# tkkiran/Robust-Conditional-GAN

Hardware: AMD Instinct MI355X
Metric: images/sec G+D train step (CIFAR-10 RCGAN bs=64) (higher is better)
Workload: dtype bf16

## Files before the change

### include/rcgan_hip.h

```cpp
#ifndef RCGAN_HIP_H
#define RCGAN_HIP_H

#include <stddef.h>
#include <stdint.h>

#ifdef __cplusplus
extern "C" {
#endif

#define RCGAN_OK 0
#define RCGAN_EINVALID_ARG (-1)
#define RCGAN_EUNSUPPORTED_SHAPE (-2)
#define RCGAN_EWORKSPACE_TOO_SMALL (-3)
#define RCGAN_EHIP (-4)
#define RCGAN_ERCCL (-5)

#define RCGAN_F32 0
#define RCGAN_BF16 1
#define RCGAN_F16 2

#define RCGAN_ACT_NONE 0
#define RCGAN_ACT_RELU 1
#define RCGAN_ACT_LRELU 2
#define RCGAN_ACT_TANH 3
// ... 217 lines not shown
int rcgan_dtrunk_prepare(rcgan_ctx* ctx, const void* const* prepared, void* frag);
int rcgan_dtrunk(rcgan_ctx* ctx, int n, int backward, const void* x0, const void* frag, const float* const* bias,
                 const void* const* masks, void* const* outs);
int rcgan_dtrunk_pooled(rcgan_ctx* ctx, int n, int backward, const void* x0, const void* frag, const float* const* bias,
                        const void* const* masks, void* const* outs, float* feat, const void* xlast, void* dy_out);

int rcgan_conv_rf_ok(const rcgan_conv_desc* d);
size_t rcgan_conv_rf_fragment_bytes(const rcgan_conv_desc* d);
int rcgan_conv_rf_prepare(rcgan_ctx* ctx, int n, const rcgan_conv_desc* descs, const void* const* prepared, void* const* frags);
int rcgan_fragments_prepare(rcgan_ctx* ctx, const void* const* trunk_prepared, void* trunk_frag, int n, const rcgan_conv_desc* descs,
                            const void* const* prepared, void* const* frags);
int rcgan_conv2d_rf(rcgan_ctx* ctx, const rcgan_conv_desc* d, int backward, const void* x, const void* frag, const float* bias,
                    const void* mask_x, const void* residual, void* y);

int rcgan_dblock2_ok(const rcgan_conv_desc* d, const void* conv1_frag, const void* dblock2_frag);
size_t rcgan_dblock2_fragment_bytes(void);
int rcgan_fragments_prepare_dblock2(rcgan_ctx* ctx, const void* const* trunk_prepared, void* trunk_frag, int n, const rcgan_conv_desc* descs,
                                    const void* const* prepared, void* const* frags, const void* conv2_prepared,
                                    const void* shortcut_prepared, void* dblock2_frag);
int rcgan_dblock2_fwd(rcgan_ctx* ctx, const rcgan_conv_desc* d, const void* x, const void* conv1_frag, const void* dblock2_frag,
                      const float* bias1, const float* bias2, const float* bias_shortcut, void* h, void* xp, void* y);
int rcgan_dblock2_bwd(rcgan_ctx* ctx, const rcgan_conv_desc* d, const void* dy, const void* h, const void* x, const void* conv1_frag,
                      const void* dblock2_frag, void* dh, void* dx);
size_t rcgan_proj_head_workspace_bytes(int n, int d, int v);
typedef struct {
  int n, d, v, e_dim;
  int rows_a, kind_a, kind_b;
  float weight;
  const int32_t* labels_a; const float* wts_a; float* dwts_a;
  const int32_t* labels_b; const float* wts_b; float* dwts_b;
  const void* x; void* dx;
  int x_dtype, hw, act;
  const float* E_pre;
  void* defer_ws;
  size_t defer_ws_bytes;
} rcgan_head_desc;
int rcgan_proj_head_fwd_bwd(rcgan_ctx* ctx, const rcgan_head_desc* hd, const float* feat, const float* w_out, const float* sigma_out,
                            const float* b_out, const float* table, const float* w_e, const float* sigma_e, const float* b_e,
                            float* loss_acc, float* logits, float* dfeat, float* dw_out, float* db_out, float* dtable, float* dw_e,
                            float* db_e, void* ws, size_t ws_bytes);
int rcgan_head_flush(rcgan_ctx* ctx);
int rcgan_bce_onehot_fwd_bwd(rcgan_ctx* ctx, int rows, int cols, const float* x, const int32_t* labels,
                             float weight, float* loss_acc, float* dx);
size_t rcgan_recover_mse_workspace_bytes(int r, int ydim);
int rcgan_recover_mse_fwd_bwd(rcgan_ctx* ctx, int r, int ydim, int pix, int dtype, const void* gen, const void* actual,
                              const float* yrec, float* loss, void* dgen, float* dyrec, void* ws, size_t ws_bytes);
// ... 116 lines not shown
```

### robust-conditional-gan_amd/_lib.py

```python
import ctypes as C
import os

_HERE = os.path.dirname(os.path.abspath(__file__))
LIB_PATH = os.environ.get("RCGAN_LIB_PATH") or os.path.join(_HERE, "librcgan_hip.so")
LIB_PATH_F16 = os.environ.get("RCGAN_LIB_PATH_F16") or os.path.join(_HERE, "librcgan_hip_f16.so")

F32, BF16, F16 = 0, 1, 2
ACT_NONE, ACT_RELU, ACT_LRELU, ACT_TANH, ACT_SIGMOID = 0, 1, 2, 3, 4
CONV_IN_UPSAMPLE2X, CONV_IN_RELU, CONV_ACCUMULATE, CONV_FORCE_DIRECT, CONV_OUT_MEANPOOL2, CONV_RESID_UPSAMPLE2X = 1, 2, 4, 8, 16, 32
LOSS_HINGE_REAL, LOSS_HINGE_FAKE, LOSS_NEG_MEAN, LOSS_CE_ONES, LOSS_CE_ZEROS = 0, 1, 2, 3, 4
QUERY_TR_READ = 0
AUG_COLOR, AUG_TRANSLATION, AUG_CUTOUT = 1, 2, 4
AUG_POLICIES = {"color": AUG_COLOR, "translation": AUG_TRANSLATION, "cutout": AUG_CUTOUT}
F32_PRECISION_HIGHEST, F32_PRECISION_HIGH = 0, 1
F32_PRECISIONS = {"highest": F32_PRECISION_HIGHEST, "high": F32_PRECISION_HIGH}

RCGAN_EHIP, RCGAN_ERCCL = -4, -5
EINVALID_ARG, EUNSUPPORTED_SHAPE, EWORKSPACE_TOO_SMALL = -1, -2, -3
ERRORS = {-1: "RCGAN_EINVALID_ARG", -2: "RCGAN_EUNSUPPORTED_SHAPE", -3: "RCGAN_EWORKSPACE_TOO_SMALL",
          -4: "RCGAN_EHIP", -5: "RCGAN_ERCCL"}


def source_hash():
    import glob
# ... 164 lines not shown
    "rcgan_act_meanhw_fwd": (I, [P, I, I, I, I, I, P, P]),
    "rcgan_act_meanhw_bwd": (I, [P, I, I, I, I, I, P, P, P]),
    "rcgan_gather_rows": (I, [P, I, I, P, P, P]),
    "rcgan_scatter_add_rows": (I, [P, I, I, I, P, P, P, I]),
    "rcgan_proj_logit_fwd": (I, [P, I, I, P, P, P, P]),
    "rcgan_proj_logit_bwd": (I, [P, I, I, P, P, P, P, P, P, I]),
    "rcgan_proj_logit_all_fwd": (I, [P, I, I, I, P, P, P, P]),
    "rcgan_proj_logit_all_bwd": (I, [P, I, I, I, P, P, P, P, P, P, I]),
    "rcgan_loss_fwd_bwd": (I, [P, I, I, I, P, P, F, P, P, P]),
    "rcgan_bce_onehot_fwd_bwd": (I, [P, I, I, P, P, F, P, P]),
    "rcgan_dtrunk": (I, [P, I, I, P, P, P, P, P]),
    "rcgan_dtrunk_pooled": (I, [P, I, I, P, P, P, P, P, P, P, P]),
    "rcgan_dtrunk_prepare": (I, [P, P, P]),
    "rcgan_conv_rf_ok": (I, [C.POINTER(ConvDesc)]),
    "rcgan_conv_rf_fragment_bytes": (SZ, [C.POINTER(ConvDesc)]),
    "rcgan_conv_rf_prepare": (I, [P, I, C.POINTER(ConvDesc), P, P]),
    "rcgan_fragments_prepare": (I, [P, P, P, I, C.POINTER(ConvDesc), P, P]),
    "rcgan_conv2d_rf": (I, [P, C.POINTER(ConvDesc), I, P, P, P, P, P, P]),
    "rcgan_dblock2_ok": (I, [C.POINTER(ConvDesc), P, P]),
    "rcgan_dblock2_fragment_bytes": (SZ, []),
    "rcgan_fragments_prepare_dblock2": (I, [P, P, P, I, C.POINTER(ConvDesc), P, P, P, P, P]),
    "rcgan_dblock2_fwd": (I, [P, C.POINTER(ConvDesc), P, P, P, P, P, P, P, P, P]),
    "rcgan_dblock2_bwd": (I, [P, C.POINTER(ConvDesc), P, P, P, P, P, P, P]),
    "rcgan_dtrunk_fragment_bytes": (SZ, []),
    "rcgan_head_flush": (I, [P]),
    "rcgan_proj_head_fwd_bwd": (I, [P, C.POINTER(HeadDesc)] + [P] * 16 + [P, SZ]),
    "rcgan_recover_mse_fwd_bwd": (I, [P, I, I, I, I, P, P, P, P, P, P, P, SZ]),
    "rcgan_softmax_rows_fwd": (I, [P, I, I, P, P]),
    "rcgan_softmax_rows_bwd": (I, [P, I, I, P, P, P, I]),
    "rcgan_softmax_xent_workspace_bytes": (SZ, [I]),
    "rcgan_softmax_xent_fwd_bwd": (I, [P, I, I, P, P, F, P, P, P, P, SZ]),
    "rcgan_softmax_xent_forward_fwd_bwd": (I, [P, I, I, P, P, P, F, P, P, P, P, P, P, SZ]),
    "rcgan_shortcut_a_fwd": (I, [P, I, I, I, I, I, P, P]),
    "rcgan_shortcut_a_bwd": (I, [P, I, I, I, I, I, P, P, I]),
    "rcgan_diffaugment_fwd": (I, [P, I, I, I, I, I, P, P, P, P]),
    "rcgan_diffaugment_bwd": (I, [P, I, I, I, I, I, P, P, P, I]),
    "rcgan_diffaugment_gated_fwd": (I, [P, I, I, I, I, I, P, P, P, P, P, P, P]),
    "rcgan_diffaugment_sampled_bwd": (I, [P, I, I, I, I, P, P, P, P, I]),
    "rcgan_ada_update": (I, [P, I, P, I, P, P, F, F, I]),
    "rcgan_class_moments_bytes": (SZ, [I, I]),
    "rcgan_class_moments_accum": (I, [P, I, I, I, P, P, P]),
    "rcgan_knn_radius": (I, [P, I, I, I, I, P, P, P]),
    "rcgan_ball_query": (I, [P, I, I, I, I, P, P, P, P, P, P, P]),
    "rcgan_poly3_rowsum": (I, [P, I, I, I, I, P, P, P, P, C.c_double, C.c_double, I, P]),
    "rcgan_msssim_pairs": (I, [P, I, I, I, I, I, P, P, P]),
    "rcgan_nn_u8": (I, [P, I, I, I, I, P, P, P, P, I, P]),
# ... 67 lines not shown
```

### robust-conditional-gan_amd/cifar.py

```python
import ctypes as C
import os

import warnings

import numpy as np
import torch

from . import _lib as L
from . import ops as O
from . import runtime
from .ops_cifar import NO_OPS, Conv2D, Linear, cond_batchnorm, embed_y, spectral_normed_weight
from .runtime import DT, Context, ParamGroup, check_f32_matmul_precision, run_rehearsed
from .variables import Graph, scoped, variable_scope

Z_DIM = 128
DIM_G = 128
DIM_D = 128
VOCAB_SIZE = 10
EMBEDDING_DIM = 300
IMG_SIZE = 32
IMG_DIM = 3
OUTPUT_DIM = 3072
N_CRITIC = 5
GEN_BS_MULTIPLE = 2
# ... 233 lines not shown
                                    _defer_apply=True)
        output = Conv2D(output, DIM_G * 2, IMG_DIM, 3, 1, 'G.Output', he_init=False)
        output = O.act(ctx, output, L.ACT_TANH, out=out.reshape(output.shape) if out is not None else None)
        return O.reshape(ctx, output, (-1, OUTPUT_DIM))


def fused_pool_d(ctx, n):
    if ctx.act_dtype == L.F32 or os.environ.get("RCGAN_FUSED_POOL", "1") != "1":
        return False
    d1 = L.ConvDesc(n, IMG_SIZE, IMG_SIZE, DIM_D, DIM_D, 3, 3, 1, ctx.act_dtype, L.CONV_OUT_MEANPOOL2)
    d2 = L.ConvDesc(n, IMG_SIZE // 2, IMG_SIZE // 2, DIM_D, DIM_D, 3, 3, 1, ctx.act_dtype, L.CONV_OUT_MEANPOOL2)
    return bool(ctx.lib.rcgan_conv_fused_pool_ok(C.byref(d1))) and bool(ctx.lib.rcgan_conv_fused_pool_ok(C.byref(d2)))


def Discriminator(inputs, labels, update_collection=None, _head=True):
    ctx = _ctx()
    kw = dict(spectral_normed=True, update_collection=update_collection)
    with variable_scope("Discriminator"):
        x = O.reshape(ctx, inputs, (-1, IMG_SIZE, IMG_SIZE, IMG_DIM))
        if fused_pool_d(ctx, x.shape[0]):
            xp = getattr(Graph.current, "image_pool", None)
            if xp is not None and (x.req or xp.shape != (x.shape[0], x.shape[1] // 2, x.shape[2] // 2, x.shape[3])):
                xp = None
            t = Conv2D(xp if xp is not None else O.meanpool2(ctx, x), IMG_DIM, DIM_D, 1, 1, 'D.Block.1.Shortcut', he_init=False, **kw)
            h = Conv2D(x, IMG_DIM, DIM_D, 3, 1, 'D.Block.1.Conv1', **kw)
            x = Conv2D(h, DIM_D, DIM_D, 3, 1, 'D.Block.1.Conv2', _in_relu=True, _accumulate_into=t, _out_meanpool=True, **kw)
            g, wb = Graph.current, []
            for cv in ('Shortcut', 'Conv1', 'Conv2'):
                with variable_scope('D.Block.2.%s' % cv):
                    fname = scoped('Filters')
                    with variable_scope('filters'):
                        wb.append(spectral_normed_weight(fname, update_collection=update_collection))
                    wb.append(g.param(scoped('Biases')))
            dfrag = getattr(g, "dblock2_frag", None)
            if O.d_block2_ok(ctx, x, wb[2], dfrag):
                x = O.d_block2(ctx, x, *wb, frag=dfrag)
            else:
                t = O.conv2d(ctx, O.meanpool2(ctx, x), wb[0], wb[1], 1)
                h = O.conv2d(ctx, x, wb[2], wb[3], 3, in_relu=True)
                x = O.conv2d_meanpool(ctx, h, wb[4], wb[5], in_relu=True, accumulate_into=t)
        else:
            t = Conv2D(x, IMG_DIM, DIM_D, 1, 1, 'D.Block.1.Shortcut', he_init=False, **kw)
            h = Conv2D(x, IMG_DIM, DIM_D, 3, 1, 'D.Block.1.Conv1', **kw)
            t = Conv2D(h, DIM_D, DIM_D, 3, 1, 'D.Block.1.Conv2', _in_relu=True, _accumulate_into=t, **kw)
            x = O.meanpool2(ctx, t)
            t = Conv2D(x, DIM_D, DIM_D, 1, 1, 'D.Block.2.Shortcut', he_init=False, **kw)
            h = Conv2D(x, DIM_D, DIM_D, 3, 1, 'D.Block.2.Conv1', _in_relu=True, **kw)
            t = Conv2D(h, DIM_D, DIM_D, 3, 1, 'D.Block.2.Conv2', _in_relu=True, _accumulate_into=t, **kw)
            x = O.meanpool2(ctx, t)
        if Graph.current.early_d is not None and x.req:
# ... 314 lines not shown
        for n in grp.names:
            if n.endswith("/Filters"):
                shp = grp.shapes[n]
                up = L.CONV_IN_UPSAMPLE2X if (n.startswith("Generator/G.Block.") and n.endswith(".Conv1/Filters")) else 0
                if pool and n in ("Discriminator/D.Block.1.Conv2/Filters", "Discriminator/D.Block.2.Conv2/Filters"):
                    up = L.CONV_OUT_MEANPOOL2
                names.append((n, shp[0], 1, IMG_SIZE if min(shp[2], shp[3]) <= 3 else 8, up))
            elif n == "Generator/G.Input/W" and O.LINEAR_MFMA:
                names.append((n, 1, 1, 1, 0))
        return names

    def _prepare_all(self, which, head_update=False, inputs=None):
        names = []
        for grp in which:
            if grp is not self.PG:
                names += self._filter_names(grp)
        g, embed = self.graph, None
        g.head_E = None
        if self.fused_head and self.PD in which and head_update is not False and self.K <= L.LABELS_NARROW and \
                os.environ.get("RCGAN_HEAD_EMBED_RIDE", "1") == "1":
            _, _, table, w_e, b_e = _head_weights(head_update)
            E = self.ctx.empty((table.shape[0], w_e.param.shape[-1]), L.F32)
            embed = (table, w_e, b_e, E)
        g.trunk_frag = g.dblock2_frag = None
        trunk, rf, db2 = None, [], None
        if self.PD in which and self.ctx.act_dtype != L.F32 and (FUSED_TRUNK or O.RF_CONV):
            sn = lambda n: g.sn["Discriminator/%s/Filters" % n][0]
            trunk = [sn("D.Block.%d.%s" % (b, c)) for b in (3, 4, 5, 6) for c in ("Conv1", "Conv2")] if FUSED_TRUNK else None
            if O.RF_CONV:
                d = L.ConvDesc(1, 16, 16, DIM_D, DIM_D, 3, 3, 1, self.ctx.act_dtype, L.CONV_IN_RELU)
                if self.ctx.lib.rcgan_conv_rf_ok(C.byref(d)):
                    rf.append((sn("D.Block.2.Conv1"), d))
                    if O.FUSED_DBLOCK2 and fused_pool_d(self.ctx, GEN_BS_MULTIPLE * self.B):
                        db2 = (sn("D.Block.2.Conv2"), sn("D.Block.2.Shortcut"))
        if (trunk or rf) and O.FRAG_IN_PREPARE:
            tf, reqs = O.fragment_requests(self.ctx, trunk, rf)
            rode, written = g.prepare_convs(names, self.ctx.act_dtype, embed=embed, inputs=inputs, frags=reqs)
            if len(written) == len(reqs):
                g.trunk_frag = tf
            else:
                g.trunk_frag = O.fragments_batch(self.ctx, trunk, rf)
        else:
            rode = g.prepare_convs(names, self.ctx.act_dtype, embed=embed, inputs=inputs)
            if db2 is not None:
                g.trunk_frag, g.dblock2_frag = O.fragments_batch(self.ctx, trunk, rf, dblock2=db2)
            elif trunk or rf:
                g.trunk_frag = O.fragments_batch(self.ctx, trunk, rf)
        if rode and embed is not None:
            g.head_E = embed[3]
        return rode

    def _refresh_generator_filters(self):
        if self._pg_prepared_version != self.PG.version:
            self.graph.refresh_persistent(self._filter_names(self.PG), self.ctx.act_dtype)
            self._pg_prepared_version = self.PG.version

    def confusion_matrix(self):
        ctx = self.ctx
        if self.PC is not None:
            return O.softmax_rows(ctx, self.graph.param("confusion_logits"))
        return self.inp["C_const"]

    def _rides_inputs(self):
        return self.device_rng and self.ride_inputs and self.PD.gradbuf.numel() % 4 == 0

    def _d_body(self, fakes_ready=False):
        ctx, g, B, inp = self.ctx, self.graph, self.B, self.inp
# ... 502 lines not shown
```

### robust-conditional-gan_amd/csrc/conv_rf.hip

```cpp
#include <type_traits>

#include "conv_mfma.h"
#include "mfma_util.h"
#include "rf_asm.h"

namespace {

struct RfArgs {
  const bf16_t* in;
  const bf16_t* wfrag;
  const float* bias;
  const bf16_t* mask;
  const bf16_t* resid;
  bf16_t* out;
  const bf16_t* zero;
  int accumulate, relu_in;
  int H, W, lbpi, Cout;
  int res_lw, res_lh;
  long M;
  unsigned long long* stamps;
};

constexpr int RF_ROWS = 8;
constexpr int RF_UPFRONT = 4;
// ... 210 lines not shown
      for (int dir = 0; dir < 2; ++dir) {
        const int K = 9 * (dir ? d->cout : d->cin), nsl = (dir ? d->cout : d->cin) / 64;
        FragItem& it = b.it[2 * i + dir];
        it.src = (const bf16_t*)prepared[i0 + i] + dir * elems;
        it.dst = (bf16_t*)frags[i0 + i] + dir * elems;
        it.K = K; it.ctn = 4; it.ss = 18; it.nsl = nsl; it.chunks = (int)(elems / 8);
        if (it.chunks > maxchunks) maxchunks = it.chunks;
      }
    }
    hipLaunchKernelGGL(rf_fragments_kernel, dim3(cdiv(maxchunks, 256), 2 * m), dim3(256), 0, ctx->stream, b);
    RC_LAUNCH_CHECK(ctx);
  }
  return RCGAN_OK;
}

int rcgan_fragments_prepare(rcgan_ctx* ctx, const void* const* trunk_prepared, void* trunk_frag, int n, const rcgan_conv_desc* descs,
                            const void* const* prepared, void* const* frags) {
  return rcgan_fragments_prepare_dblock2(ctx, trunk_prepared, trunk_frag, n, descs, prepared, frags, nullptr, nullptr, nullptr);
}

int rcgan_fragments_prepare_dblock2(rcgan_ctx* ctx, const void* const* trunk_prepared, void* trunk_frag, int n, const rcgan_conv_desc* descs,
                                    const void* const* prepared, void* const* frags, const void* conv2_prepared,
                                    const void* shortcut_prepared, void* dblock2_frag) {
  if (!ctx) return RCGAN_EINVALID_ARG;
  RC_REQUIRE(ctx, n >= 0 && n <= 12 && (n == 0 || (descs && prepared && frags)) && (!trunk_prepared || trunk_frag), "bad arguments");
  RC_REQUIRE(ctx, (conv2_prepared != nullptr) == (dblock2_frag != nullptr) && (shortcut_prepared != nullptr) == (dblock2_frag != nullptr),
             "the down block's copies need both prepared filters and a destination");
  RC_REQUIRE(ctx, (dblock2_frag ? DB2_FRAG_ITEMS : 0) + (trunk_prepared ? 16 : 0) + 2 * n <= (int)(sizeof(FragBatch::it) / sizeof(FragItem)),
             "more fragment items than one launch holds");
  FragBatch b;
  int m = 0, maxchunks = 0;
  if (dblock2_frag) {
    const rcgan_conv_desc d2 = {1, 16, 16, 128, 128, 3, 3, 1, RCGAN_H16, RCGAN_CONV_OUT_MEANPOOL2};
    const rcgan_conv_desc ds = {1, 8, 8, 128, 128, 1, 1, 1, RCGAN_H16, 0};
    dblock2_frag_items((const bf16_t*)conv2_prepared + mfma_prepared_sum_fwd(&d2), (const bf16_t*)shortcut_prepared,
                       (const bf16_t*)conv2_prepared + mfma_prepared_sum_bwd(&d2), (const bf16_t*)shortcut_prepared + mfma_prepared_rot(&ds),
                       (bf16_t*)dblock2_frag, b.it);
    m = DB2_FRAG_ITEMS;
    maxchunks = b.it[0].chunks;
  }
  if (trunk_prepared) {
    const long elems = 9L * 128 * 128;
    for (int i = 0; i < 8; ++i) {
      RC_REQUIRE(ctx, trunk_prepared[i], "stage layer %d: null pointer", i);
      b.it[m++] = FragItem{(const bf16_t*)trunk_prepared[i], (bf16_t*)trunk_frag + i * elems, 1152, 2, 36, 1, (int)(elems / 8)};
      b.it[m++] = FragItem{(const bf16_t*)trunk_prepared[7 - i] + elems, (bf16_t*)trunk_frag + (8 + i) * elems, 1152, 2, 36, 1, (int)(elems / 8)};
    }
    if ((int)(elems / 8) > maxchunks) maxchunks = (int)(elems / 8);
  }
  for (int i = 0; i < n; ++i) {
    const rcgan_conv_desc* d = descs + i;
    RC_REQUIRE(ctx, rf_takes(d) && prepared[i] && frags[i], "filter %d: not a register-filter shape / null pointer", i);
    const long elems = 9L * d->cin * d->cout;
    for (int dir = 0; dir < 2; ++dir) {
      const int kc = dir ? d->cout : d->cin;
      b.it[m++] = FragItem{(const bf16_t*)prepared[i] + dir * elems, (bf16_t*)frags[i] + dir * elems, 9 * kc, 4, 18, kc / 64, (int)(elems / 8)};
    }
    if ((int)(elems / 8) > maxchunks) maxchunks = (int)(elems / 8);
  }
  if (m == 0) return RCGAN_OK;
  hipLaunchKernelGGL(rf_fragments_kernel, dim3(cdiv(maxchunks, 256), m), dim3(256), 0, ctx->stream, b);
  RC_LAUNCH_CHECK(ctx);
// ... 31 lines not shown
```

### robust-conditional-gan_amd/csrc/rf_asm.h

```cpp
#pragma once
#include <type_traits>

#include "mfma_util.h"

typedef __attribute__((ext_vector_type(4))) int i32x4_t;

#if RCGAN_HALF_FP16
#define RF_MFMA "v_mfma_f32_16x16x32_f16"
#else
#define RF_MFMA "v_mfma_f32_16x16x32_bf16"
#endif

template <int OFF> __device__ __forceinline__ void rf_load_a(i32x4_t& dst, const void* p) {
  asm volatile("global_load_dwordx4 %0, %1, off offset:%2" : "=a"(dst) : "v"(p), "n"(OFF) : "memory");
}
template <int OFF> __device__ __forceinline__ void rf_load_v(i32x4_t& dst, const void* p) {
  asm volatile("global_load_dwordx4 %0, %1, off offset:%2" : "=v"(dst) : "v"(p), "n"(OFF) : "memory");
}
template <int OFF> __device__ __forceinline__ void rf_load_a_inplace(i32x4_t& dst, const void* p) {
  asm volatile("global_load_dwordx4 %0, %1, off offset:%2" : "+a"(dst) : "v"(p), "n"(OFF) : "memory");
}
__device__ __forceinline__ void rf_mfma_a(f32x4_t& acc, const i32x4_t& w, const bf16x8_t& x) {
  asm volatile(RF_MFMA " %0, %1, %2, %0" : "+v"(acc) : "a"(w), "v"(x) : "memory");
}
__device__ __forceinline__ void rf_mfma_v(f32x4_t& acc, const i32x4_t& w, const bf16x8_t& x) {
  asm volatile(RF_MFMA " %0, %1, %2, %0" : "+v"(acc) : "v"(w), "v"(x) : "memory");
}
__device__ __forceinline__ void rf_mfma_a0(f32x4_t& acc, const i32x4_t& w, const bf16x8_t& x) {
  asm volatile(RF_MFMA " %0, %1, %2, 0" : "=v"(acc) : "a"(w), "v"(x) : "memory");
}
__device__ __forceinline__ void rf_lds_read(bf16x8_t& dst, unsigned lds_byte_addr) {
  asm volatile("ds_read_b128 %0, %1" : "=v"(dst) : "v"(lds_byte_addr) : "memory");
}
template <int N> __device__ __forceinline__ void rf_wait() { asm volatile("s_waitcnt vmcnt(%0)" :: "n"(N) : "memory"); }
__device__ __forceinline__ void rf_barrier() { asm volatile("s_waitcnt lgkmcnt(0)\n\ts_barrier" ::: "memory"); }

template <int I, int N, typename F> __device__ __forceinline__ void rf_for(F&& f) {
  if constexpr (I < N) { f(std::integral_constant<int, I>{}); rf_for<I + 1, N>(f); }
}

struct FragItem { const bf16_t* src; bf16_t* dst; int K, ctn, ss, nsl, chunks; };

constexpr long DB2_FRAG_CONV2 = 16L * 128 * 128;
constexpr long DB2_FRAG_SHORT = 128L * 128;
constexpr long DB2_FRAG_CONV2_BWD = DB2_FRAG_CONV2 + DB2_FRAG_SHORT;
constexpr long DB2_FRAG_SHORT_BWD = DB2_FRAG_CONV2_BWD + DB2_FRAG_CONV2;
constexpr long DB2_FRAG_ELEMS = DB2_FRAG_SHORT_BWD + DB2_FRAG_SHORT;
constexpr int DB2_FRAG_ITEMS = 4;
inline void dblock2_frag_items(const bf16_t* conv2_sum_fwd, const bf16_t* shortcut_fwd, const bf16_t* conv2_sum_bwd, const bf16_t* shortcut_rot,
                               bf16_t* frag, FragItem* it) {
  it[0] = FragItem{conv2_sum_fwd, frag, 2048, 2, 64, 1, (int)(DB2_FRAG_CONV2 / 8)};
  it[1] = FragItem{shortcut_fwd, frag + DB2_FRAG_CONV2, 128, 2, 4, 1, (int)(DB2_FRAG_SHORT / 8)};
  it[2] = FragItem{conv2_sum_bwd, frag + DB2_FRAG_CONV2_BWD, 512, 2, 16, 1, (int)(DB2_FRAG_CONV2 / 8)};
  it[3] = FragItem{shortcut_rot, frag + DB2_FRAG_SHORT_BWD, 128, 2, 4, 1, (int)(DB2_FRAG_SHORT / 8)};
}
```

### robust-conditional-gan_amd/ops.py

```python
import ctypes as C
import os

import torch

from . import _lib as L
from .runtime import DT


def _p(t):
    return C.c_void_p(t.ptr) if t is not None else None


def same_pad(n, k, s):
    out = -(-n // s)
    tot = max((out - 1) * s + k - n, 0)
    return out, tot // 2


def zeros_like_grad(ctx, t):
    g = ctx.empty(t.shape, t.dtype)
    ctx.check(ctx.lib.rcgan_fill_f32(ctx.h, (g.nbytes + 3) // 4, g.ptr, 0.0))
    return g


# ... 119 lines not shown
CONCAT_DIRECT = os.environ.get("RCGAN_CONCAT_DIRECT", "1") != "0"
CONCAT_WGRAD = os.environ.get("RCGAN_CONCAT_WGRAD", "1") != "0"
LINEAR_MFMA = os.environ.get("RCGAN_LINEAR_MFMA", "1") != "0"


FRAG_IN_PREPARE = os.environ.get("RCGAN_FRAG_IN_PREPARE", "0") == "1"


def fragment_requests(ctx, trunk, rf):
    reqs, tf = [], None
    if trunk:
        nb = ctx.lib.rcgan_dtrunk_fragment_bytes()
        tf = DT(ctx.arena.alloc(nb), (nb,), "u8", ctx.arena.buf)
        elems2 = 9 * 128 * 128 * 2
        for i, w in enumerate(trunk):
            reqs.append((w, tf.ptr + i * elems2, tf.ptr + (8 + (7 - i)) * elems2, 2, 36))
    for w, d in rf:
        nb = ctx.lib.rcgan_conv_rf_fragment_bytes(C.byref(d))
        w.rf_frag = DT(ctx.arena.alloc(nb), (nb,), "u8", ctx.arena.buf)
        reqs.append((w, w.rf_frag.ptr, w.rf_frag.ptr + nb // 2, 4, 18))
    return tf, reqs


def fragments_batch(ctx, trunk, rf, dblock2=None):
    tp = tf = None
    if trunk:
        tdesc = L.ConvDesc(1, 8, 8, 128, 128, 3, 3, 1, ctx.act_dtype, L.CONV_IN_RELU)
        tp = (C.c_void_p * 8)(*[w.prepared(tdesc).ptr for w in trunk])
        nb = ctx.lib.rcgan_dtrunk_fragment_bytes()
        tf = DT(ctx.arena.alloc(nb), (nb,), "u8", ctx.arena.buf)
    n = len(rf)
    descs = (L.ConvDesc * max(n, 1))(*[d for _, d in rf])
    preps = (C.c_void_p * max(n, 1))(*[w.prepared(d).ptr for w, d in rf])
    frags = []
    for w, d in rf:
        nb = ctx.lib.rcgan_conv_rf_fragment_bytes(C.byref(d))
        w.rf_frag = DT(ctx.arena.alloc(nb), (nb,), "u8", ctx.arena.buf)
        frags.append(w.rf_frag.ptr)
    if dblock2 is not None:
        w2, ws = dblock2
        p2 = w2.prepared(L.ConvDesc(1, 8, 8, 128, 128, 3, 3, 1, ctx.act_dtype, L.CONV_OUT_MEANPOOL2))
        ps = ws.prepared(L.ConvDesc(1, 8, 8, 128, 128, 1, 1, 1, ctx.act_dtype, 0))
        nb = ctx.lib.rcgan_dblock2_fragment_bytes()
        df = DT(ctx.arena.alloc(nb), (nb,), "u8", ctx.arena.buf)
        ctx.check(ctx.lib.rcgan_fragments_prepare_dblock2(ctx.h, tp, _p(tf), n, descs, preps, (C.c_void_p * max(n, 1))(*frags),
                                                          _p(p2), _p(ps), _p(df)))
        return tf, df
    ctx.check(ctx.lib.rcgan_fragments_prepare(ctx.h, tp, _p(tf), n, descs, preps, (C.c_void_p * max(n, 1))(*frags)))
    return tf


def spectral_norm_batch(ctx, entries):
    n = len(entries)
    if n == 0:
        return []
    items = (L.SnItem * n)()
    weights = []
    saves = []
    for i, (param, u, update) in enumerate(entries):
        c = param.shape[-1]
        k = param.size // c
        sigma = ctx.empty((1,), L.F32)
        save = ctx.empty((ctx.lib.rcgan_sn_save_floats(k, c),), L.F32)
        items[i] = L.SnItem(param.ptr, u.ptr, sigma.ptr, save.ptr, k, c, 1 if update else 0)
        weights.append(Weight(ctx, param, sigma))
        saves.append((save, k, c))
    ctx.check(ctx.lib.rcgan_sn_power_iter(ctx.h, items, n))
# ... 277 lines not shown
            dy = out.grad
            if dy is None:
                return
            fused = (x.req and x.grad is None and ctx.group_wgrads and h.grad is None and xp.grad is None
                     and not (ctx.overlap and wreq[1])
                     and all(wr or not b.req for wr, (_, _, _, b) in zip(wreq, layers))
                     and (not wreq[0] or ctx.lib.rcgan_conv_wgrad_pool_ok(C.byref(d2))))
            if not fused:
                for fn in reversed(four):
                    fn()
                return
            dh, dx = d_block2_bwd(ctx, d, dy, h, x, w1, frag)
            for wr, (desc, operand, w, b), g in zip(wreq, layers, (dy, dh, dy)):
                if wr:
                    ctx.defer_wgrad(desc, operand, g, w.grad_target(), b.grad if b.req else None)
            h.grad = dh
            x.grad = dx
        ctx.record(bw)
    return out


FUSED_DBLOCK2_BWD = os.environ.get("RCGAN_FUSED_DBLOCK2_BWD", "1") != "0"


def d_trunk_ok(ctx, x):
    return x.dtype != L.F32 and tuple(x.shape[1:]) == (8, 8, 128)


def d_trunk(ctx, x, blocks, pool=None, frag=None):
    n = x.shape[0]
    assert d_trunk_ok(ctx, x) and len(blocks) == 4 and pool in (None, L.ACT_RELU)
    desc = L.ConvDesc(n, 8, 8, 128, 128, 3, 3, 1, x.dtype, L.CONV_IN_RELU)
    arr = lambda ts: (C.c_void_p * 8)(*[(t.ptr if t is not None else None) for t in ts])
    flat = []
    for w1, b1, w2, b2 in blocks:
        flat += [(w1, b1), (w2, b2)]
    preps = [w.prepared(desc) for w, _ in flat]
    outs = [ctx.empty(x.shape, x.dtype) for _ in range(8)]
    if frag is None:
        frag = DT(ctx.arena.alloc(ctx.lib.rcgan_dtrunk_fragment_bytes()), (ctx.lib.rcgan_dtrunk_fragment_bytes(),), "u8", ctx.arena.buf)
        ctx.check(ctx.lib.rcgan_dtrunk_prepare(ctx.h, arr(preps), _p(frag)))
    feat = ctx.empty((n, 128), L.F32) if pool is not None else None
    ctx.check(ctx.lib.rcgan_dtrunk_pooled(ctx.h, n, 0, _p(x), _p(frag), arr([b for _, b in flat]), None, arr(outs), _p(feat), None, None))
    y = outs[7]
    y.pooled, y.pool_grad = ((feat, pool) if feat is not None else None), None
    params = [t for w, b in flat for t in (w.param, b)]
# ... 741 lines not shown
```

Before: 63940.

## Fuse discriminator input block forward into one register-resident MFMA kernel

Adds a fused HIP kernel for the discriminator's first residual block on 32x32x3 input. A single launch per image band computes Conv1, ReLU, Conv2 with meanpool, the pooled-input shortcut and both biases, keeping the Conv1 output in LDS and streaming Conv2 weights through an AccVGPR ring from a pre-copied fragment. The goal is to remove several separate launches and the HBM round trip of the intermediate activation. In exchange it adds fragment preparation, a new code path gated by an environment flag and shape checks, and it still writes h for the backward pass.

New measurement: 65010 (median of 6 runs). 1.02x the previous value.

```diff
diff --git a/include/rcgan_hip.h b/include/rcgan_hip.h
--- a/include/rcgan_hip.h
+++ b/include/rcgan_hip.h
@@ -263,6 +263,14 @@
                       const float* bias1, const float* bias2, const float* bias_shortcut, void* h, void* xp, void* y);
 int rcgan_dblock2_bwd(rcgan_ctx* ctx, const rcgan_conv_desc* d, const void* dy, const void* h, const void* x, const void* conv1_frag,
                       const void* dblock2_frag, void* dh, void* dx);
+
+int rcgan_dblock1_ok(const rcgan_conv_desc* d, const void* dblock1_frag);
+size_t rcgan_dblock1_fragment_bytes(void);
+int rcgan_fragments_prepare_dblocks(rcgan_ctx* ctx, const void* const* trunk_prepared, void* trunk_frag, int n, const rcgan_conv_desc* descs,
+                                    const void* const* prepared, void* const* frags, const void* conv2_prepared,
+                                    const void* shortcut_prepared, void* dblock2_frag, const void* block1_conv2_prepared, void* dblock1_frag);
+int rcgan_dblock1_fwd(rcgan_ctx* ctx, const rcgan_conv_desc* d, const void* x, const void* conv1_prepared, const void* shortcut_prepared,
+                      const void* dblock1_frag, const float* bias1, const float* bias2, const float* bias_shortcut, void* h, void* xp, void* y);
 size_t rcgan_proj_head_workspace_bytes(int n, int d, int v);
 typedef struct {
   int n, d, v, e_dim;
diff --git a/robust-conditional-gan_amd/_lib.py b/robust-conditional-gan_amd/_lib.py
--- a/robust-conditional-gan_amd/_lib.py
+++ b/robust-conditional-gan_amd/_lib.py
@@ -210,6 +210,10 @@
     "rcgan_fragments_prepare_dblock2": (I, [P, P, P, I, C.POINTER(ConvDesc), P, P, P, P, P]),
     "rcgan_dblock2_fwd": (I, [P, C.POINTER(ConvDesc), P, P, P, P, P, P, P, P, P]),
     "rcgan_dblock2_bwd": (I, [P, C.POINTER(ConvDesc), P, P, P, P, P, P, P]),
+    "rcgan_dblock1_ok": (I, [C.POINTER(ConvDesc), P]),
+    "rcgan_dblock1_fragment_bytes": (SZ, []),
+    "rcgan_fragments_prepare_dblocks": (I, [P, P, P, I, C.POINTER(ConvDesc), P, P, P, P, P, P, P]),
+    "rcgan_dblock1_fwd": (I, [P, C.POINTER(ConvDesc), P, P, P, P, P, P, P, P, P, P]),
     "rcgan_dtrunk_fragment_bytes": (SZ, []),
     "rcgan_head_flush": (I, [P]),
     "rcgan_proj_head_fwd_bwd": (I, [P, C.POINTER(HeadDesc)] + [P] * 16 + [P, SZ]),
diff --git a/robust-conditional-gan_amd/cifar.py b/robust-conditional-gan_amd/cifar.py
--- a/robust-conditional-gan_amd/cifar.py
+++ b/robust-conditional-gan_amd/cifar.py
@@ -279,10 +279,22 @@
             xp = getattr(Graph.current, "image_pool", None)
             if xp is not None and (x.req or xp.shape != (x.shape[0], x.shape[1] // 2, x.shape[2] // 2, x.shape[3])):
                 xp = None
-            t = Conv2D(xp if xp is not None else O.meanpool2(ctx, x), IMG_DIM, DIM_D, 1, 1, 'D.Block.1.Shortcut', he_init=False, **kw)
-            h = Conv2D(x, IMG_DIM, DIM_D, 3, 1, 'D.Block.1.Conv1', **kw)
-            x = Conv2D(h, DIM_D, DIM_D, 3, 1, 'D.Block.1.Conv2', _in_relu=True, _accumulate_into=t, _out_meanpool=True, **kw)
-            g, wb = Graph.current, []
+            g = Graph.current
+            d1frag = getattr(g, "dblock1_frag", None)
+            if O.d_block1_ok(ctx, x, d1frag):
+                wb = []
+                for cv in ('Shortcut', 'Conv1', 'Conv2'):
+                    with variable_scope('D.Block.1.%s' % cv):
+                        fname = scoped('Filters')
+                        with variable_scope('filters'):
+                            wb.append(spectral_normed_weight(fname, update_collection=update_collection))
+                        wb.append(g.param(scoped('Biases')))
+                x = O.d_block1(ctx, x, *wb, frag=d1frag, pooled=xp)
+            else:
+                t = Conv2D(xp if xp is not None else O.meanpool2(ctx, x), IMG_DIM, DIM_D, 1, 1, 'D.Block.1.Shortcut', he_init=False, **kw)
+                h = Conv2D(x, IMG_DIM, DIM_D, 3, 1, 'D.Block.1.Conv1', **kw)
+                x = Conv2D(h, DIM_D, DIM_D, 3, 1, 'D.Block.1.Conv2', _in_relu=True, _accumulate_into=t, _out_meanpool=True, **kw)
+            wb = []
             for cv in ('Shortcut', 'Conv1', 'Conv2'):
                 with variable_scope('D.Block.2.%s' % cv):
                     fname = scoped('Filters')
@@ -643,10 +655,12 @@
             _, _, table, w_e, b_e = _head_weights(head_update)
             E = self.ctx.empty((table.shape[0], w_e.param.shape[-1]), L.F32)
             embed = (table, w_e, b_e, E)
-        g.trunk_frag = g.dblock2_frag = None
-        trunk, rf, db2 = None, [], None
+        g.trunk_frag = g.dblock2_frag = g.dblock1_frag = None
+        trunk, rf, db2, db1 = None, [], None, None
         if self.PD in which and self.ctx.act_dtype != L.F32 and (FUSED_TRUNK or O.RF_CONV):
             sn = lambda n: g.sn["Discriminator/%s/Filters" % n][0]
+            if O.FUSED_DBLOCK1 and fused_pool_d(self.ctx, GEN_BS_MULTIPLE * self.B):
+                db1 = sn("D.Block.1.Conv2")
             trunk = [sn("D.Block.%d.%s" % (b, c)) for b in (3, 4, 5, 6) for c in ("Conv1", "Conv2")] if FUSED_TRUNK else None
             if O.RF_CONV:
                 d = L.ConvDesc(1, 16, 16, DIM_D, DIM_D, 3, 3, 1, self.ctx.act_dtype, L.CONV_IN_RELU)
@@ -663,7 +677,9 @@
                 g.trunk_frag = O.fragments_batch(self.ctx, trunk, rf)
         else:
             rode = g.prepare_convs(names, self.ctx.act_dtype, embed=embed, inputs=inputs)
-            if db2 is not None:
+            if db1 is not None:
+                g.trunk_frag, g.dblock2_frag, g.dblock1_frag = O.fragments_batch(self.ctx, trunk, rf, dblock2=db2, dblock1=db1)
+            elif db2 is not None:
                 g.trunk_frag, g.dblock2_frag = O.fragments_batch(self.ctx, trunk, rf, dblock2=db2)
             elif trunk or rf:
                 g.trunk_frag = O.fragments_batch(self.ctx, trunk, rf)
diff --git a/robust-conditional-gan_amd/csrc/conv_dblock1.hip b/robust-conditional-gan_amd/csrc/conv_dblock1.hip
--- /dev/null
+++ b/robust-conditional-gan_amd/csrc/conv_dblock1.hip
@@ -0,0 +1,250 @@
+#include "conv_mfma.h"
+#include "mfma_util.h"
+#include "rf_asm.h"
+
+namespace {
+
+constexpr int D1_PW = 34;
+constexpr int D1_XROWS = 12;
+constexpr int D1_XELEMS = D1_XROWS * D1_PW * 3;
+constexpr int D1_XBYTES = (D1_XELEMS * 2 + 16 + 255) / 256 * 256;
+constexpr int D1_HROWS = 10;
+constexpr int D1_HNPP = D1_HROWS * D1_PW;
+constexpr int D1_HBYTES = D1_HNPP * 256;
+constexpr int D1_XPBYTES = 64 * 4 * 2;
+constexpr int D1_BIAS = 3 * 128 * 4;
+constexpr int D1_LDS = D1_XBYTES + D1_HBYTES + D1_XPBYTES + D1_BIAS;
+constexpr int D1_RING = 32;
+constexpr int D1_STEPS2 = 64;
+static_assert(D1_LDS <= 160 * 1024, "LDS of one CU");
+static_assert(D1_STEPS2 % D1_RING == 0 && D1_RING * 8 == 256, "the ring is the 256 AccVGPRs");
+
+struct Db1Args {
+  const bf16_t* x;
+  const bf16_t* wk1;
+  const bf16_t* wks;
+  const bf16_t* w2;
+  const float *b1, *b2, *bs;
+  bf16_t *h, *xp, *y;
+  unsigned long long* stamps;
+};
+
+__global__ __launch_bounds__(256) void conv_dblock1_kernel(Db1Args a) {
+  extern __shared__ __attribute__((aligned(16))) unsigned char smem[];
+  const int tid = threadIdx.x, lane = tid & 63;
+  const int wave = __builtin_amdgcn_readfirstlane(tid >> 6);
+  const int r = lane & 15, kc = lane >> 4;
+  const int n = (int)blockIdx.x >> 2, band = (int)blockIdx.x & 3;
+  bf16_t* const xs = (bf16_t*)smem;
+  unsigned char* const himg = smem + D1_XBYTES;
+  bf16_t* const xps = (bf16_t*)(himg + D1_HBYTES);
+  float* const bias_s = (float*)(himg + D1_HBYTES + D1_XPBYTES);
+  auto stamp = [&](int k) __attribute__((always_inline)) {
+    if (a.stamps && tid == 0) a.stamps[(long)blockIdx.x * 16 + k] = __builtin_amdgcn_s_memtime();
+  };
+  stamp(0);
+
+  const bf16_t* const img = a.x + (long)n * (32 * 32 * 3);
+  for (int e = tid; e < D1_XELEMS + 8; e += 256) {
+    bf16_t v = 0;
+    if (e < D1_XELEMS) {
+      const int pr = e / (D1_PW * 3), rem = e - pr * (D1_PW * 3), pc = rem / 3, c = rem - pc * 3;
+      const int ih = 8 * band - 2 + pr, iw = pc - 1;
+      if (ih >= 0 && ih < 32 && iw >= 0 && iw < 32) v = img[(ih * 32 + iw) * 3 + c];
+    }
+    xs[e] = v;
+  }
+  if (tid < 96) *(float4*)(bias_s + tid * 4) = *(const float4*)((tid < 32 ? a.b1 : tid < 64 ? a.b2 : a.bs) + (tid & 31) * 4);
+  bf16x8_t wf[8], wsf[2];
+#pragma unroll
+  for (int i = 0; i < 8; ++i) {
+    const int ch = (i >> 1) * 32 + (r >> 2) * 8 + (i & 1) * 4 + (r & 3);
+    wf[i] = *(const bf16x8_t*)(a.wk1 + ch * 32 + kc * 8);
+  }
+#pragma unroll
+  for (int ct = 0; ct < 2; ++ct) wsf[ct] = *(const bf16x8_t*)(a.wks + (wave * 32 + ct * 16 + r) * 32 + kc * 8);
+  for (int i = tid; i < 2 * D1_HROWS * 16; i += 256) {
+    const int p = i >> 4, pp = (p >> 1) * D1_PW + (p & 1) * (D1_PW - 1);
+    ((uint4*)(himg + pp * 256))[i & 15] = make_uint4(0u, 0u, 0u, 0u);
+  }
+  if (band == 0 || band == 3) {
+    uint4* const row = (uint4*)(himg + (band ? (D1_HROWS - 1) * D1_PW * 256 : 0));
+    for (int i = tid; i < D1_PW * 16; i += 256) row[i] = make_uint4(0u, 0u, 0u, 0u);
+  }
+  __syncthreads();
+#pragma unroll
+  for (int i = 0; i < 8; ++i) asm volatile("" : "+v"(wf[i]));
+#pragma unroll
+  for (int ct = 0; ct < 2; ++ct) asm volatile("" : "+v"(wsf[ct]));
+  stamp(1);
+
+  i32x4_t WA[D1_RING / 2][4];
+  const bf16_t* const w2c = a.w2 + (long)wave * (D1_STEPS2 * 1024) + lane * 8;
+  rf_for<0, D1_RING>([&](auto ic) __attribute__((always_inline)) {
+    constexpr int u = decltype(ic)::value;
+    rf_load_a<0>(WA[u >> 1][2 * (u & 1)], w2c + u * 1024); rf_load_a<1024>(WA[u >> 1][2 * (u & 1) + 1], w2c + u * 1024);
+  });
+  auto w2load = [&](auto ic) __attribute__((always_inline)) {
+    constexpr int u = decltype(ic)::value, slot = u % D1_RING;
+    const bf16_t* const p = w2c + u * 1024;
+    rf_load_a_inplace<0>(WA[slot >> 1][2 * (slot & 1)], p); rf_load_a_inplace<1024>(WA[slot >> 1][2 * (slot & 1) + 1], p);
+  };
+
+  if (tid < 192) {
+    const int p = tid / 3, c = tid - p * 3, pi = p >> 4, pj = p & 15;
+    const int e00 = ((2 + 2 * pi) * D1_PW + 1 + 2 * pj) * 3 + c;
+    const float v = (((bf16_to_f32(xs[e00]) + bf16_to_f32(xs[e00 + D1_PW * 3])) + bf16_to_f32(xs[e00 + 3])) + bf16_to_f32(xs[e00 + D1_PW * 3 + 3])) * 0.25f;
+    const bf16_t o = f32_to_bf16(v);
+    xps[p * 4 + c] = o;
+    if (a.xp) a.xp[(((long)n * 16 + 4 * band + pi) * 16 + pj) * 3 + c] = o;
+  } else {
+    xps[(tid - 192) * 4 + 3] = 0;
+  }
+
+  int koff[8];
+#pragma unroll
+  for (int e = 0; e < 8; ++e) {
+    const int k = kc * 8 + e, tap = k / 3, c = k - tap * 3, kh = tap / 3, kw = tap - kh * 3;
+    koff[e] = k < 27 ? (kh * D1_PW + kw) * 3 + c : -1;
+  }
+  for (int t = wave; t < 2 * D1_HROWS; t += 4) {
+    const int hr = t >> 1, col = (t & 1) * 16 + r;
+    const int ih = 8 * band - 1 + hr;
+    if (ih < 0 || ih >= 32) continue;
+    const int base = (hr * D1_PW + col) * 3;
+    uint32_t v[8];
+#pragma unroll
+    for (int e = 0; e < 8; ++e) v[e] = xs[koff[e] >= 0 ? base + koff[e] : D1_XELEMS];
+    const bf16x8_t xf = __builtin_bit_cast(bf16x8_t, make_uint4(v[0] | (v[1] << 16), v[2] | (v[3] << 16), v[4] | (v[5] << 16), v[6] | (v[7] << 16)));
+    const int pp = hr * D1_PW + col + 1;
+    const bool own = hr >= 1 && hr <= 8;
+    bf16_t* const orow = a.h + (((long)n * 32 + ih) * 32 + col) * 128 + kc * 8;
+    f32x4_t lo[4], hi[4];
+    asm volatile("s_nop 1" ::: "memory");
+#pragma unroll
+    for (int q = 0; q < 4; ++q) { rf_mfma_vv0(lo[q], wf[2 * q], xf); rf_mfma_vv0(hi[q], wf[2 * q + 1], xf); }
+    asm volatile("s_nop 15\n\ts_nop 15" ::: "memory");
+#pragma unroll
+    for (int q = 0; q < 4; ++q) {
+      const float4 ba = *(const float4*)(bias_s + q * 32 + kc * 8), bb = *(const float4*)(bias_s + q * 32 + kc * 8 + 4);
+      uint4 pk;
+      pk.x = pack_h16x2(lo[q][0] + ba.x, lo[q][1] + ba.y);
+      pk.y = pack_h16x2(lo[q][2] + ba.z, lo[q][3] + ba.w);
+      pk.z = pack_h16x2(hi[q][0] + bb.x, hi[q][1] + bb.y);
+      pk.w = pack_h16x2(hi[q][2] + bb.z, hi[q][3] + bb.w);
+      if (own) *(uint4*)(orow + q * 32) = pk;
+      pk.x = relu_bf16x2(pk.x); pk.y = relu_bf16x2(pk.y); pk.z = relu_bf16x2(pk.z); pk.w = relu_bf16x2(pk.w);
+      *(uint4*)(himg + pp * 256 + (((q * 4 + kc) ^ ((pp >> 1) & 15)) << 4)) = pk;
+    }
+  }
+  stamp(2);
+  asm volatile("s_waitcnt vmcnt(0)" ::: "memory");
+  rf_barrier();
+  stamp(3);
+
+  int rr = r;
+  asm volatile("" : "+v"(rr));
+  auto xread = [&](auto ic, bf16x8_t (&xf)[4]) __attribute__((always_inline)) {
+    constexpr int u = decltype(ic)::value, tap = u >> 2, cq = u & 3, uu = tap >> 2, vv = tap & 3;
+#pragma unroll
+    for (int pt = 0; pt < 4; ++pt) {
+      const int pp = (2 * pt + uu) * D1_PW + vv + 2 * rr;
+      xf[pt] = *(const bf16x8_t*)(himg + pp * 256 + (((cq * 4 + kc) ^ ((pp >> 1) & 15)) << 4));
+    }
+  };
+  f32x4_t acc2[4][2];
+  bf16x8_t xf2[2][4];
+  xread(std::integral_constant<int, 0>{}, xf2[0]);
+  rf_for<0, D1_STEPS2>([&](auto ic) __attribute__((always_inline)) {
+    constexpr int u = decltype(ic)::value, slot = u % D1_RING;
+    if constexpr (u + 1 < D1_STEPS2) xread(std::integral_constant<int, u + 1>{}, xf2[(u + 1) & 1]);
+    rf_wait<2 * ((u + D1_RING - 1 < D1_STEPS2 - 1 ? u + D1_RING - 1 : D1_STEPS2 - 1) - u)>();
+#pragma unroll
+    for (int ct = 0; ct < 2; ++ct)
+#pragma unroll
+      for (int pt = 0; pt < 4; ++pt) {
+        const i32x4_t& w = WA[slot >> 1][2 * (slot & 1) + ct];
+        if constexpr (u == 0) rf_mfma_a0e(acc2[pt][ct], w, xf2[u & 1][pt]);
+        else rf_mfma_a(acc2[pt][ct], w, xf2[u & 1][pt]);
+      }
+    if constexpr (u + D1_RING < D1_STEPS2) w2load(std::integral_constant<int, u + D1_RING>{});
+  });
+  stamp(4);
+  asm volatile("s_nop 15\n\ts_nop 15" ::: "memory");
+  f32x4_t accs[4][2];
+  bf16x8_t xpf[4];
+#pragma unroll
+  for (int pt = 0; pt < 4; ++pt) {
+    const uint2 xv = *(const uint2*)(xps + (pt * 16 + r) * 4);
+    xpf[pt] = __builtin_bit_cast(bf16x8_t, kc == 0 ? make_uint4(xv.x, xv.y, 0u, 0u) : make_uint4(0u, 0u, 0u, 0u));
+    asm volatile("" : "+v"(xpf[pt]));
+  }
+  asm volatile("s_nop 1" ::: "memory");
+#pragma unroll
+  for (int pt = 0; pt < 4; ++pt)
+#pragma unroll
+    for (int ct = 0; ct < 2; ++ct) rf_mfma_vv0(accs[pt][ct], wsf[ct], xpf[pt]);
+  asm volatile("s_nop 15\n\ts_nop 15" ::: "memory");
+#pragma unroll
+  for (int pt = 0; pt < 4; ++pt) {
+#pragma unroll
+    for (int ct = 0; ct < 2; ++ct) {
+      const f32x4_t s = accs[pt][ct];
+      const int c0 = wave * 32 + ct * 16 + 4 * kc;
+      const float4 b2 = *(const float4*)(bias_s + 128 + c0), bs = *(const float4*)(bias_s + 256 + c0);
+      uint2 t;
+      t.x = pack_h16x2(s[0] + bs.x, s[1] + bs.y);
+      t.y = pack_h16x2(s[2] + bs.z, s[3] + bs.w);
+      const f32x4_t c2 = acc2[pt][ct];
+      uint2 pk;
+      pk.x = pack_h16x2((c2[0] + b2.x) + h16_lo(t.x), (c2[1] + b2.y) + h16_hi(t.x));
+      pk.y = pack_h16x2((c2[2] + b2.z) + h16_lo(t.y), (c2[3] + b2.w) + h16_hi(t.y));
+      *(uint2*)(a.y + (((long)n * 16 + 4 * band + pt) * 16 + r) * 128 + c0) = pk;
+    }
+  }
+  if (a.stamps) {
+    asm volatile("s_waitcnt vmcnt(0)" ::: "memory");
+    stamp(5);
+  }
+}
+
+bool dblock1_takes(const rcgan_conv_desc* d) {
+  if (!d || d->dtype != RCGAN_H16 || d->kh != 3 || d->kw != 3 || d->stride != 1 || d->flags != 0) return false;
+  if (!(d->n >= 1 && d->h == 32 && d->w == 32 && d->cin == 3 && d->cout == 128)) return false;
+  return (long)d->n * d->h * d->w * d->cout < (1L << 31);
+}
+
+}
+
+extern "C" {
+
+int rcgan_dblock1_ok(const rcgan_conv_desc* d, const void* dblock1_frag) { return dblock1_takes(d) && dblock1_frag ? 1 : 0; }
+
+size_t rcgan_dblock1_fragment_bytes(void) { return (size_t)DB1_FRAG_ELEMS * sizeof(bf16_t); }
+
+int rcgan_dblock1_fwd(rcgan_ctx* ctx, const rcgan_conv_desc* d, const void* x, const void* conv1_prepared, const void* shortcut_prepared,
+                      const void* dblock1_frag, const float* bias1, const float* bias2, const float* bias_shortcut, void* h, void* xp, void* y) {
+  if (!ctx) return RCGAN_EINVALID_ARG;
+  RC_REQUIRE(ctx, rcgan_dblock1_ok(d, dblock1_frag), "not the 32x32x3 input block / missing fragment copy (rcgan_dblock1_ok)");
+  RC_REQUIRE(ctx, x && conv1_prepared && shortcut_prepared && bias1 && bias2 && bias_shortcut && h && y, "null argument");
+  const rcgan_conv_desc ds = {d->n, 16, 16, 3, 128, 1, 1, 1, d->dtype, 0};
+  RC_REQUIRE(ctx, img_side(d) == 1 && img_side(&ds) == 1, "the image-end rows of Conv1 and the shortcut are not prepared for this build");
+  Db1Args a;
+  a.x = (const bf16_t*)x;
+  a.wk1 = (const bf16_t*)((const char*)conv1_prepared + img_extra_offset(d));
+  a.wks = (const bf16_t*)((const char*)shortcut_prepared + img_extra_offset(&ds));
+  a.w2 = (const bf16_t*)dblock1_frag;
+  a.b1 = bias1; a.b2 = bias2; a.bs = bias_shortcut;
+  a.h = (bf16_t*)h; a.xp = (bf16_t*)xp; a.y = (bf16_t*)y;
+  a.stamps = (unsigned long long*)ctx->dbg_stamps;
+  static bool attr_set = false;
+  if (!attr_set) {
+    RC_HIP(ctx, hipFuncSetAttribute((const void*)conv_dblock1_kernel, hipFuncAttributeMaxDynamicSharedMemorySize, (int)D1_LDS));
+    attr_set = true;
+  }
+  hipLaunchKernelGGL(conv_dblock1_kernel, dim3(4 * d->n), dim3(256), D1_LDS, ctx->stream, a);
+  RC_LAUNCH_CHECK(ctx);
+  return RCGAN_OK;
+}
+
+}
diff --git a/robust-conditional-gan_amd/csrc/conv_rf.hip b/robust-conditional-gan_amd/csrc/conv_rf.hip
--- a/robust-conditional-gan_amd/csrc/conv_rf.hip
+++ b/robust-conditional-gan_amd/csrc/conv_rf.hip
@@ -256,11 +256,20 @@
 int rcgan_fragments_prepare_dblock2(rcgan_ctx* ctx, const void* const* trunk_prepared, void* trunk_frag, int n, const rcgan_conv_desc* descs,
                                     const void* const* prepared, void* const* frags, const void* conv2_prepared,
                                     const void* shortcut_prepared, void* dblock2_frag) {
+  return rcgan_fragments_prepare_dblocks(ctx, trunk_prepared, trunk_frag, n, descs, prepared, frags, conv2_prepared, shortcut_prepared, dblock2_frag,
+                                         nullptr, nullptr);
+}
+
+int rcgan_fragments_prepare_dblocks(rcgan_ctx* ctx, const void* const* trunk_prepared, void* trunk_frag, int n, const rcgan_conv_desc* descs,
+                                    const void* const* prepared, void* const* frags, const void* conv2_prepared,
+                                    const void* shortcut_prepared, void* dblock2_frag, const void* block1_conv2_prepared, void* dblock1_frag) {
   if (!ctx) return RCGAN_EINVALID_ARG;
+  RC_REQUIRE(ctx, (block1_conv2_prepared != nullptr) == (dblock1_frag != nullptr), "the input block's copy needs its prepared filter and a destination");
   RC_REQUIRE(ctx, n >= 0 && n <= 12 && (n == 0 || (descs && prepared && frags)) && (!trunk_prepared || trunk_frag), "bad arguments");
   RC_REQUIRE(ctx, (conv2_prepared != nullptr) == (dblock2_frag != nullptr) && (shortcut_prepared != nullptr) == (dblock2_frag != nullptr),
              "the down block's copies need both prepared filters and a destination");
-  RC_REQUIRE(ctx, (dblock2_frag ? DB2_FRAG_ITEMS : 0) + (trunk_prepared ? 16 : 0) + 2 * n <= (int)(sizeof(FragBatch::it) / sizeof(FragItem)),
+  RC_REQUIRE(ctx, (dblock2_frag ? DB2_FRAG_ITEMS : 0) + (dblock1_frag ? DB1_FRAG_ITEMS : 0) + (trunk_prepared ? 16 : 0) + 2 * n <=
+                      (int)(sizeof(FragBatch::it) / sizeof(FragItem)),
              "more fragment items than one launch holds");
   FragBatch b;
   int m = 0, maxchunks = 0;
@@ -272,6 +281,12 @@
                        (bf16_t*)dblock2_frag, b.it);
     m = DB2_FRAG_ITEMS;
     maxchunks = b.it[0].chunks;
+  }
+  if (dblock1_frag) {
+    const rcgan_conv_desc d2 = {1, 32, 32, 128, 128, 3, 3, 1, RCGAN_H16, RCGAN_CONV_OUT_MEANPOOL2};
+    dblock1_frag_items((const bf16_t*)block1_conv2_prepared + mfma_prepared_sum_fwd(&d2), (bf16_t*)dblock1_frag, b.it + m);
+    if (b.it[m].chunks > maxchunks) maxchunks = b.it[m].chunks;
+    m += DB1_FRAG_ITEMS;
   }
   if (trunk_prepared) {
     const long elems = 9L * 128 * 128;
diff --git a/robust-conditional-gan_amd/csrc/rf_asm.h b/robust-conditional-gan_amd/csrc/rf_asm.h
--- a/robust-conditional-gan_amd/csrc/rf_asm.h
+++ b/robust-conditional-gan_amd/csrc/rf_asm.h
@@ -29,6 +29,12 @@
 __device__ __forceinline__ void rf_mfma_a0(f32x4_t& acc, const i32x4_t& w, const bf16x8_t& x) {
   asm volatile(RF_MFMA " %0, %1, %2, 0" : "=v"(acc) : "a"(w), "v"(x) : "memory");
 }
+__device__ __forceinline__ void rf_mfma_a0e(f32x4_t& acc, const i32x4_t& w, const bf16x8_t& x) {
+  asm volatile(RF_MFMA " %0, %1, %2, 0" : "=&v"(acc) : "a"(w), "v"(x) : "memory");
+}
+__device__ __forceinline__ void rf_mfma_vv0(f32x4_t& acc, const bf16x8_t& w, const bf16x8_t& x) {
+  asm volatile("s_nop 4\n\t" RF_MFMA " %0, %1, %2, 0" : "=&v"(acc) : "v"(w), "v"(x) : "memory");
+}
 __device__ __forceinline__ void rf_lds_read(bf16x8_t& dst, unsigned lds_byte_addr) {
   asm volatile("ds_read_b128 %0, %1" : "=v"(dst) : "v"(lds_byte_addr) : "memory");
 }
@@ -54,3 +60,9 @@
   it[2] = FragItem{conv2_sum_bwd, frag + DB2_FRAG_CONV2_BWD, 512, 2, 16, 1, (int)(DB2_FRAG_CONV2 / 8)};
   it[3] = FragItem{shortcut_rot, frag + DB2_FRAG_SHORT_BWD, 128, 2, 4, 1, (int)(DB2_FRAG_SHORT / 8)};
 }
+
+constexpr long DB1_FRAG_ELEMS = 16L * 128 * 128;
+constexpr int DB1_FRAG_ITEMS = 1;
+inline void dblock1_frag_items(const bf16_t* conv2_sum_fwd, bf16_t* frag, FragItem* it) {
+  it[0] = FragItem{conv2_sum_fwd, frag, 2048, 2, 64, 1, (int)(DB1_FRAG_ELEMS / 8)};
+}
diff --git a/robust-conditional-gan_amd/ops.py b/robust-conditional-gan_amd/ops.py
--- a/robust-conditional-gan_amd/ops.py
+++ b/robust-conditional-gan_amd/ops.py
@@ -165,7 +165,7 @@
     return tf, reqs
 
 
-def fragments_batch(ctx, trunk, rf, dblock2=None):
+def fragments_batch(ctx, trunk, rf, dblock2=None, dblock1=None):
     tp = tf = None
     if trunk:
         tdesc = L.ConvDesc(1, 8, 8, 128, 128, 3, 3, 1, ctx.act_dtype, L.CONV_IN_RELU)
@@ -180,12 +180,21 @@
         nb = ctx.lib.rcgan_conv_rf_fragment_bytes(C.byref(d))
         w.rf_frag = DT(ctx.arena.alloc(nb), (nb,), "u8", ctx.arena.buf)
         frags.append(w.rf_frag.ptr)
+    p2 = ps = df = None
     if dblock2 is not None:
         w2, ws = dblock2
         p2 = w2.prepared(L.ConvDesc(1, 8, 8, 128, 128, 3, 3, 1, ctx.act_dtype, L.CONV_OUT_MEANPOOL2))
         ps = ws.prepared(L.ConvDesc(1, 8, 8, 128, 128, 1, 1, 1, ctx.act_dtype, 0))
         nb = ctx.lib.rcgan_dblock2_fragment_bytes()
         df = DT(ctx.arena.alloc(nb), (nb,), "u8", ctx.arena.buf)
+    if dblock1 is not None:
+        p1 = dblock1.prepared(L.ConvDesc(1, 8, 8, 128, 128, 3, 3, 1, ctx.act_dtype, L.CONV_OUT_MEANPOOL2))
+        nb = ctx.lib.rcgan_dblock1_fragment_bytes()
+        d1f = DT(ctx.arena.alloc(nb), (nb,), "u8", ctx.arena.buf)
+        ctx.check(ctx.lib.rcgan_fragments_prepare_dblocks(ctx.h, tp, _p(tf), n, descs, preps, (C.c_void_p * max(n, 1))(*frags),
+                                                          _p(p2), _p(ps), _p(df), _p(p1), _p(d1f)))
+        return tf, df, d1f
+    if dblock2 is not None:
         ctx.check(ctx.lib.rcgan_fragments_prepare_dblock2(ctx.h, tp, _p(tf), n, descs, preps, (C.c_void_p * max(n, 1))(*frags),
                                                           _p(p2), _p(ps), _p(df)))
         return tf, df
@@ -509,6 +518,33 @@
 
 FUSED_DBLOCK2_BWD = os.environ.get("RCGAN_FUSED_DBLOCK2_BWD", "1") != "0"
 
+FUSED_DBLOCK1 = os.environ.get("RCGAN_FUSED_DBLOCK1", "1") != "0"
+
+
+def d_block1_ok(ctx, x, frag):
+    if not FUSED_DBLOCK1 or frag is None or len(x.shape) != 4 or x.dtype == L.F32:
+        return False
+    n, h, w, c = x.shape
+    d = L.ConvDesc(n, h, w, c, 128, 3, 3, 1, x.dtype, 0)
+    return bool(ctx.lib.rcgan_dblock1_ok(C.byref(d), _p(frag)))
+
+
+def d_block1(ctx, x, ws, bs, w1, b1, w2, b2, frag, pooled=None, _saved=None):
+    n = x.shape[0]
+    d = L.ConvDesc(n, 32, 32, 3, 128, 3, 3, 1, x.dtype, 0)
+    ds = L.ConvDesc(n, 16, 16, 3, 128, 1, 1, 1, x.dtype, 0)
+    h = ctx.empty((n, 32, 32, 128), x.dtype)
+    y = ctx.empty((n, 16, 16, 128), x.dtype)
+    xp = ctx.empty((n, 16, 16, 3), x.dtype) if pooled is None else None
+    ctx.check(ctx.lib.rcgan_dblock1_fwd(ctx.h, C.byref(d), _p(x), _p(w1.prepared(d)), _p(ws.prepared(ds)), _p(frag), _p(b1), _p(b2), _p(bs),
+                                        _p(h), _p(xp), _p(y)))
+    xp = pooled if pooled is not None else meanpool2(ctx, x, _done=xp)
+    t = conv2d(ctx, xp, ws, bs, 1, _done=y)
+    h = conv2d(ctx, x, w1, b1, 3, _done=h)
+    if _saved is not None:
+        _saved += [h, xp]
+    return conv2d_meanpool(ctx, h, w2, b2, in_relu=True, accumulate_into=t, _done=True)
+
 
 def d_trunk_ok(ctx, x):
     return x.dtype != L.F32 and tuple(x.shape[1:]) == (8, 8, 128)
```
